# psweens/VAN-GAN

Measured on AMD Instinct MI355X. Metric: train Mvoxels/s (VanGan.train_step, 128^3 bf16), higher is better.
Workload: dtype bf16; 1 GPU; VanGan.train_step, 128x128x128 volumes, batch 1 per GPU (global 1), clDice on, disc noise+dropout on; parallelism=dp1

## Files before the change

van_gan_amd/csrc/vg_conv_common.h:

```cpp
#pragma once
#include "vg_gather.h"

struct ConvOut {
    int OD, OH, OW, ostr, ood, ooh, oow, BD, BH, BW, Cout;
    const void* wp; int Ktot, nchunks, kc_pad;
    const float* bias; const void* res; const float* rs; const float* rb; int tanh_out;
    int res1;
    int wdma;
    const void* wp_up; int nup;
    void* out; int out_f32, accumulate; float* sums;
    int w_lds;
    int dma;
    int xw;
    int dbg;
    int WRS;
    const void* bs_x0; const void* bs_x1; int bs_c0, bs_sh, bs_act, bs_pad, bs_D, bs_H, bs_W;
    const float* bs_sc; const float* bs_sf; const float* bs_mu; const float* bs_rs; const float* bs_ml;
    int ks; float* ks_part; unsigned* ks_cnt;
    char* scratch; long scratch_bytes;
    VgFin fin;
};
struct ConvCls {
    int ncls;
    int par;
// ... 97 lines not shown
            o1 = koff[min(s + 3, last) * 4 + kg];
            a0 = wfrag(min(s + 2, last));
#pragma unroll
            for (int i = 0; i < MW; ++i) b0[i] = *(const bf16x8*)(halo + rowbase[i] + o2);
            if (s + 1 >= ksteps) a1 = zero8;
            __builtin_amdgcn_sched_barrier(0);
#pragma unroll
            for (int i = 0; i < MW; ++i) acc[i] = VG_MFMA16(a1, b1[i], acc[i]);
            __builtin_amdgcn_sched_barrier(0);
        }
    }
}


bool vg_conv_thin_ok(const vg_conv_desc* d, const GatherIn& g, const ConvOut& k, const ConvCls& q, int np);
int vg_conv_thin_lds_bytes(const GatherIn& g, int np, int pl = 1, bool up = false, bool wdma = false);
int vg_launch_conv_thin(const GatherIn& g, const ConvOut& k, int np, hipStream_t s, float* red, bool& did_stats);
```

van_gan_amd/csrc/vg_conv_thin.hip:

```cpp
#include "vg_conv_common.h"
#include <stdio.h>

static int vg_ablate_knob(const char* key) {
    const int v = vg_tune(key, 0);
#ifdef VG_DEBUG_ABLATE
    return v;
#else
    if (v != 0) { fprintf(stderr, "libvangan_hip: VG_%s=%d is a timing-ablation knob of a -DVG_DEBUG_ABLATE build; this library refuses it\n", key, v); return -1; }
    return 0;
#endif
}
#include "vg_dma_common.h"
#include <type_traits>
#include <algorithm>
#include <cstdio>

#ifndef VG_THIN_WPE
#define VG_THIN_WPE 2
#endif
#ifndef VG_THIN_PF2
#define VG_THIN_PF2 0
#endif
#ifndef VG_THIN_PD
#define VG_THIN_PD 1
#endif
namespace {
constexpr int TW = 16, TH = 8, TD = 4;
constexpr int HW = 18, HH = 10, HD = 6;
constexpr int UNIT = 16;
constexpr int ROWB = HW * UNIT;
constexpr int DSB = HH * ROWB;
constexpr int PSB = ((HD * DSB + 255) / 256) * 256;
constexpr int HALO = 2 * PSB;
constexpr int KSTEPS = 14;
constexpr int KCPAD = 448;
}

__device__ __forceinline__ void lds_only_barrier() { asm volatile("s_waitcnt lgkmcnt(0)\n\ts_barrier" ::: "memory"); }

struct ThinItem { int hoff, cg; bool cv; const char* pc; const int* dt; };
struct ThinTab { const int* tab; int AL, NH, NW, od0, oh0, ow0; };
__device__ __forceinline__ void thin_axis_tables(const GatherIn& g, int* tab, int NH, int NW, int ND, int tid) {
    const int AL = NH + NW + ND, sh = g.shift0;
    for (int i = tid; i < 2 * AL; i += 256) {
        const int set = i >= AL ? 1 : 0, j = i - set * AL;
        if (set == 1 && g.c1 == 0) { tab[i] = -1; continue; }
        const int axis = j < NH ? 1 : (j < NH + NW ? 2 : 0);
        const int jj = axis == 1 ? j : (axis == 2 ? j - NH : j - NH - NW);
        const int n_ax = axis == 1 ? g.H : (axis == 2 ? g.W : g.D);
        int p = (axis == 1 ? g.tmin_h : (axis == 2 ? g.tmin_w : g.tmin_d)) + jj;
        const bool valid = resolve_pos(p, n_ax, g.pad_mode);
        long off;
        if (set == 0) {
            const int ps = p >> sh, Ws = g.W >> sh, Hs = g.H >> sh;
            off = axis == 1 ? (long)ps * Ws * g.c0 : (axis == 2 ? (long)ps * g.c0 : (long)ps * Hs * Ws * g.c0);
        } else off = axis == 1 ? (long)p * g.W * g.c1 : (axis == 2 ? (long)p * g.c1 : (long)p * g.H * g.W * g.c1);
        tab[i] = valid ? (int)(off * 2) : -1;
    }
}
template <bool PLAIN>
__device__ __forceinline__ ThinItem thin_item(const GatherIn& g, const int* ctab, const ThinTab& tt, const char* b0, const char* b1, int chunk, int item) {
    constexpr int NCOLS = HH * HW * 2, SEGL = HD / 2;
    ThinItem t;
    const int seg = item >= NCOLS ? 1 : 0, col = item - seg * NCOLS;
    const int e = ctab[2 * col];
    t.hoff = ctab[2 * col + 1] + seg * SEGL * DSB;
    const int hh = e & 1023, hw = (e >> 10) & 1023;
    t.cg = e >> 20;
    const int c = chunk * 16 + t.cg * 8;
    const bool from0 = c < g.c0;
    const int* rs = tt.tab + (from0 ? 0 : tt.AL);
    const int oh = rs[tt.oh0 + hh], ow = rs[tt.NH + tt.ow0 + hw];
    t.cv = !PLAIN || (c < g.Cin && (oh | ow) >= 0);
    t.pc = t.cv ? (from0 ? b0 + (size_t)c * 2 : b1 + (size_t)(c - g.c0) * 2) + (oh + ow) : b0;
    t.dt = rs + tt.NH + tt.NW + tt.od0 + seg * SEGL;
    return t;
}
template <int MODE>
__device__ __forceinline__ void thin_issue(const GatherIn& g, const int* ctab, const ThinTab& rt, int n, int chunk, int tid, Raw8<bf16_t> (&raw)[3][HD / 2]) {
    typedef bf16_t T;
    constexpr int NITEMS = 4 * HH * HW, SEGL = HD / 2;
    const int sh = g.shift0;
    const char* b0 = (const char*)g.src0 + (size_t)n * (g.D >> sh) * (g.H >> sh) * (g.W >> sh) * g.c0 * 2;
    const char* b1 = (const char*)g.src1 + (size_t)n * g.D * g.H * g.W * g.c1 * 2;
#pragma unroll
    for (int i = 0; i < 3; ++i) {
        const int item = tid + 256 * i;
        if (i < 2 || item < NITEMS) {
            const ThinItem t = thin_item<MODE == VG_STAGE_PLAIN>(g, ctab, rt, b0, b1, chunk, item);
#pragma unroll
            for (int k = 0; k < SEGL; ++k) raw_load(raw[i][k], (const T*)(t.pc + (unsigned)max(t.dt[k], 0)));
        }
    }
}
template <int MODE>
__device__ __forceinline__ void thin_commit(const GatherIn& g, char* halo, const float* scs, const int* ctab, const ThinTab& rt, int chunk, int tid,
                                            Raw8<bf16_t> (&raw)[3][HD / 2]) {
    typedef bf16_t T;
    constexpr bool plain = MODE == VG_STAGE_PLAIN;
    constexpr int NITEMS = 4 * HH * HW, SEGL = HD / 2;
#pragma unroll
    for (int i = 0; i < 3; ++i) {
        const int item = tid + 256 * i;
        if (i < 2 || item < NITEMS) {
            const ThinItem t = thin_item<plain>(g, ctab, rt, nullptr, nullptr, chunk, item);
            f32x2 sc[4], sf[4];
            if (!plain) {
#pragma unroll
                for (int j = 0; j < 4; ++j) {
                    sc[j] = (f32x2){scs[t.cg * 8 + 2 * j], scs[t.cg * 8 + 2 * j + 1]};
                    sf[j] = (f32x2){scs[16 + t.cg * 8 + 2 * j], scs[16 + t.cg * 8 + 2 * j + 1]};
                }
            }
#pragma unroll
            for (int k = 0; k < SEGL; ++k) {
                T* dst = (T*)(halo + t.hoff + k * DSB);
                if (plain) {
                    Raw8<T> r = raw[i][k];
                    raw_mask(r, t.cv && t.dt[k] >= 0);
                    *(Raw8<T>*)dst = r;
// ... 76 lines not shown
            for (int k = 0; k < 2; ++k) {
                float x[8];
                raw_unpack(raw[i][k], x);
#pragma unroll
                for (int j = 0; j < 4; ++j) {
                    f32x2 v = {x[2 * j], x[2 * j + 1]};
                    v = v * sc[j] + sf[j];
                    x[2 * j] = fmaxf(v[0], 0.f); x[2 * j + 1] = fmaxf(v[1], 0.f);
                }
                store8<bf16_t>((bf16_t*)(halo + hoff + k * DSB), x);
            }
        }
    }
}

template <int MODE, bool BIAS, bool RES, bool STATS, bool BSTAT = false, int NP = 1, int PL = 1, bool UP = false>
__global__ __launch_bounds__(256, VG_THIN_WPE) void conv_thin_kernel(const GatherIn g, const ConvOut p) {
    static_assert(PL == 1 || (NP == 1 && MODE == VG_STAGE_PLAIN && !BIAS && !RES && !STATS), "panel loop: plain data gradient only");
    static_assert(!UP || (MODE == VG_STAGE_RELU && !RES && !BSTAT && PL == 1 && NP == 1), "collapsed upsampled chunks: the decoder's first convolution, forward, one panel");
    typedef bf16_t T;
    extern __shared__ __attribute__((aligned(16))) char smem[];
    const int tid = threadIdx.x, lane = tid & 63, wave = __builtin_amdgcn_readfirstlane(tid >> 6);
    const int li = lane & 15, kg = lane >> 4;
    const int n = blockIdx.z, ntile = blockIdx.y;
    char* halo = smem;
    float* scs = (float*)(smem + HALO);
    float* stat = scs + 32;
    float* bsc = stat + 32 * NP * PL;
    float* ebs = bsc + 64 * NP * PL;
    int* tapb = (int*)(ebs + (NP > 1 ? 48 * NP : 0));
    int* utab = tapb + 32;
    constexpr int NCOLS = HH * HW * 2;
    int* xtab = utab + 2 * NCOLS;
    const int NHt = g.tiles_h * TH + 2, NWt = g.tiles_w * TW + 2, NDt = g.tiles_d * TD + 2;
    const int NHl = UP ? g.tiles_h * (TH / 2) + 2 : 0, NDl = UP ? g.tiles_d * (TD / 2) + 2 : 0;
    int* lowtab = xtab + 2 * (NHt + NWt + NDt);
    int* utu = lowtab + NHl + NDl;
    char* wlds = (char*)(utu + (UP ? 2 * UPCOLS + 16 : 0));
    const bool wdma = MODE == VG_STAGE_RELU && NP == 1 && PL == 1 && !UP && p.wdma;
    wlds = (char*)(((size_t)wlds + ((PL > 1 || wdma) ? 1023 : 15)) & ~(size_t)((PL > 1 || wdma) ? 1023 : 15));
    const int Ktot = p.Ktot, nchunks = p.nchunks;
    constexpr int WRS = KCPAD * 2 + 16;
    const int cop = ntile * 16 * NP * PL;

    build_column_table(g, utab, tid);
    if (tid < 32 * NP * PL) stat[tid] = 0.f;
    if constexpr (NP > 1 && (BIAS || RES)) {
        if (tid < 16 * NP) {
            const int c = cop + tid;
            ebs[tid] = BIAS ? p.bias[c] : 0.f;
            if (RES) { ebs[16 * NP + tid] = p.rs[n * p.Cout + c]; ebs[32 * NP + tid] = p.rb[n * p.Cout + c]; }
        }
    }
    if constexpr (BSTAT) {
        constexpr int CW = 16 * NP * PL;
        if (tid < CW) {
            const int nc = n * p.Cout + cop + tid;
            const float rs = p.bs_rs[nc];
            bsc[tid] = p.bs_sc[nc]; bsc[CW + tid] = p.bs_sf[nc]; bsc[2 * CW + tid] = rs; bsc[3 * CW + tid] = -p.bs_mu[nc] * rs;
        }
    }
    if (tid < 27) tapb[tid] = (g.td[tid] - g.tmin_d) * DSB + (g.th[tid] - g.tmin_h) * ROWB + (g.tw[tid] - g.tmin_w) * UNIT;
    auto load_weights = [&](int chunk) {
        const char* src = (const char*)p.wp + ((size_t)cop * Ktot + (size_t)chunk * KCPAD) * 2;
        constexpr int NU = 16 * NP * 56, NK = (NU + 255) / 256;
        f32x4 v[NK];
        int tid = threadIdx.x;
        if constexpr (UP) asm volatile("" : "+v"(tid));
#pragma unroll
        for (int k = 0; k < NK; ++k) {
            const int u = min(tid + k * 256, NU - 1);
            const int r = u / 56, c = u - r * 56;
            v[k] = *(const __attribute__((address_space(1))) f32x4*)(uintptr_t)(src + (size_t)r * Ktot * 2 + c * 16);
        }
#pragma unroll
        for (int k = 0; k < NK; ++k) {
            const int u = tid + k * 256;
// ... 15 lines not shown
    };
    if constexpr (PL > 1) dma_weights(0, 0); else if constexpr (!UP) { if (wdma) dma_weights(0, 0, 0); else load_weights(0); }
    const int wbase = li * WRS + kg * 16;
    const int wbase_up = li * WRSU + kg * 16;
    const int co0 = cop + 4 * kg;
    float s1[NP * PL][4], s2[NP * PL][4];
    f32x2 e_b[NP][2], e_rs[NP][2], e_rb[NP][2];
#pragma unroll
    for (int q = 0; q < NP * PL; ++q)
#pragma unroll
        for (int r = 0; r < 4; ++r) { s1[q][r] = 0.f; s2[q][r] = 0.f; }
#pragma unroll
    for (int q = 0; q < NP; ++q) {
        const int c = co0 + 16 * q;
        e_b[q][0] = (f32x2){0.f, 0.f}; e_b[q][1] = e_b[q][0];
        if (BIAS && NP == 1) { e_b[q][0] = (f32x2){p.bias[c], p.bias[c + 1]}; e_b[q][1] = (f32x2){p.bias[c + 2], p.bias[c + 3]}; }
        if (RES && NP == 1) {
            e_rs[q][0] = (f32x2){p.rs[n * p.Cout + c], p.rs[n * p.Cout + c + 1]}; e_rs[q][1] = (f32x2){p.rs[n * p.Cout + c + 2], p.rs[n * p.Cout + c + 3]};
            e_rb[q][0] = (f32x2){p.rb[n * p.Cout + c], p.rb[n * p.Cout + c + 1]}; e_rb[q][1] = (f32x2){p.rb[n * p.Cout + c + 2], p.rb[n * p.Cout + c + 3]};
        }
    }
    const T* b_x[NP]; int b_cs[NP], b_sh[NP]; float b_slope = 1.f;
#pragma unroll
    for (int q = 0; q < NP; ++q) { b_x[q] = nullptr; b_cs[q] = 0; b_sh[q] = 0; }
    auto bstat_panel = [&](const int pn16) {
#pragma unroll
        for (int q = 0; q < NP; ++q) {
            const int c = co0 + 16 * q + pn16;
            const bool lo = c < p.bs_c0;
            b_sh[q] = lo ? p.bs_sh : 0; b_cs[q] = lo ? p.bs_c0 : p.Cout - p.bs_c0;
            b_x[q] = (lo ? (const T*)p.bs_x0 + c : (const T*)p.bs_x1 + (c - p.bs_c0))
                     + (size_t)n * (p.bs_D >> b_sh[q]) * (p.bs_H >> b_sh[q]) * (p.bs_W >> b_sh[q]) * b_cs[q];
// ... 5 lines not shown
    }
    const int cst = cop + 8 * (kg >> 1);
    const int jodd = kg & 1;

    const int tiles_per_n = g.tiles_d * g.tiles_h * g.tiles_w;
    int t0 = blockIdx.x, tstep = gridDim.x, tend = tiles_per_n;
    if (p.xw) {
        const int slab = (tiles_per_n + 7) >> 3, xcd = blockIdx.x & 7;
        t0 = xcd * slab + ((int)blockIdx.x >> 3); tstep = gridDim.x >> 3; tend = min(tiles_per_n, (xcd + 1) * slab);
    }
    int gs_w, gs_h, gs_d;
    { int t = tstep; gs_w = t % g.tiles_w; t /= g.tiles_w; gs_h = t % g.tiles_h; gs_d = t / g.tiles_h; }
    int ti_w, ti_h, ti_d;
    { int t = t0; ti_w = t % g.tiles_w; t /= g.tiles_w; ti_h = t % g.tiles_h; ti_d = t / g.tiles_h; }
    if (nchunks == 1) stage_scale_shift(g, scs, n, 0, tid);
    thin_axis_tables(g, xtab, NHt, NWt, NDt, tid);
    if constexpr (UP) { build_up_table(utu, tid); thin_up_axis_tables(g, lowtab, NHl, NDl, tid); }
    lds_only_barrier();
    auto tabat = [&](int od0_, int oh0_, int ow0_) { return ThinTab{xtab, NHt + NWt + NDt, NHt, NWt, od0_, oh0_, ow0_}; };
    int boff[KSTEPS];
    {
        const int rowbase = wave * DSB + li * UNIT;
#pragma unroll
        for (int s = 0; s < KSTEPS; ++s) {
            int G = 4 * s + kg; if (G > 53) G = 53;
            boff[s] = rowbase + tapb[G >> 1] + (G & 1) * PSB;
        }
    }

    int* tapu = utu + 2 * UPCOLS;
    if constexpr (UP) { if (tid < 12) { const int cdh = tid / 3, cw = tid - cdh * 3; tapu[tid] = (cdh >> 1) * DSB + (cdh & 1) * ROWB + cw * UNIT; } }
    const int pd_cls = UP ? (wave & 1) * 2 : 0;
    constexpr int CLSB = 16 * NP * WRSU;
    auto load_weights_up = [&](int chunk) {
        const char* src = (const char*)p.wp_up + ((size_t)chunk * 4 * p.Cout + cop) * KUP * 2;
        constexpr int NU = 4 * 16 * NP * 24, NK = (NU + 255) / 256;
        f32x4 v[NK];
// ... 6 lines not shown
            v[k] = *(const __attribute__((address_space(1))) f32x4*)(uintptr_t)(src + ((size_t)cls * p.Cout + rr) * KUP * 2 + c * 16);
        }
#pragma unroll
        for (int k = 0; k < NK; ++k) {
            const int u = tl + k * 256;
            if (u < NU) { const int r = u / 24, c = u - r * 24; *(f32x4*)(wlds + r * WRSU + c * 16) = v[k]; }
        }
    };
    auto uptab = [&](int od0_, int oh0_, int ow0_) { return ThinUpTab{xtab + NHt + ow0_, lowtab + (oh0_ >> 1), lowtab + NHl + (od0_ >> 1)}; };
    typedef const __attribute__((address_space(3))) bf16x8 lds_frag;
    int it = 0;
    constexpr bool PF = MODE == VG_STAGE_RELU && (NP == 1 || VG_THIN_PF2);
    Raw8<T> raw[3][HD / 2];
    if (PF && t0 < tend) {
        if constexpr (UP) thin_issue_up<MODE>(g, utu, uptab(ti_d * TD, ti_h * TH, ti_w * TW), n, 0, tid, raw);
        else thin_issue<MODE>(g, utab, tabat(ti_d * TD, ti_h * TH, ti_w * TW), n, 0, tid, raw);
    }
    bf16x4 bxp[(BSTAT && NP == 1) ? 8 : 1];
    bf16x4 bxn[(BSTAT && PL > 1) ? 8 : 1];
    for (int tile = t0; tile < tend; tile += tstep, ++it) {
        const int od0 = ti_d * TD, oh0 = ti_h * TH, ow0 = ti_w * TW;
        ti_w += gs_w; if (ti_w >= g.tiles_w) { ti_w -= g.tiles_w; ++ti_h; }
        ti_h += gs_h; if (ti_h >= g.tiles_h) { ti_h -= g.tiles_h; ++ti_d; }
        ti_d += gs_d;
        const bool more = tile + tstep < tend;
        f32x4 acc[NP][8];
#pragma unroll
        for (int q = 0; q < NP; ++q)
#pragma unroll
            for (int j = 0; j < 8; ++j) acc[q][j] = (f32x4){0.f, 0.f, 0.f, 0.f};
        auto issue_bxp = [&]() {
// ... 45 lines not shown
                __builtin_amdgcn_sched_barrier(0);
            }
        };
        if constexpr (PL == 1)
        for (int chunk = 0; chunk < nchunks; ++chunk) {
            const bool upc = UP && chunk < p.nup;
            if (it | chunk) lds_only_barrier();
            if (nchunks > 1) {
                stage_scale_shift(g, scs, n, chunk, tid);
                if constexpr (UP) { if (upc) load_weights_up(chunk); else load_weights(chunk); }
                else if ((it | chunk) && !wdma) load_weights(chunk);
                lds_only_barrier();
            }
            if constexpr (UP) {
                if (upc) { if (!PF) thin_issue_up<MODE>(g, utu, uptab(od0, oh0, ow0), n, chunk, tid, raw); thin_commit_up(halo, scs, utu, tid, raw); }
                else { if (!PF) thin_issue<MODE>(g, utab, tabat(od0, oh0, ow0), n, chunk, tid, raw); thin_commit<MODE>(g, halo, scs, utab, tabat(od0, oh0, ow0), chunk, tid, raw); }
            } else {
            if (!PF) thin_issue<MODE>(g, utab, tabat(od0, oh0, ow0), n, chunk, tid, raw);
            thin_commit<MODE>(g, halo, scs, utab, tabat(od0, oh0, ow0), chunk, tid, raw);
            }
            if (wdma) __builtin_amdgcn_s_waitcnt(0x0F70);
            lds_only_barrier();
            if (PF) {
                if constexpr (UP) {
                    if (chunk + 1 < nchunks) {
                        if (chunk + 1 < p.nup) thin_issue_up<MODE>(g, utu, uptab(od0, oh0, ow0), n, chunk + 1, tid, raw);
                        else thin_issue<MODE>(g, utab, tabat(od0, oh0, ow0), n, chunk + 1, tid, raw);
                    } else if (more) thin_issue_up<MODE>(g, utu, uptab(ti_d * TD, ti_h * TH, ti_w * TW), n, 0, tid, raw);
                } else {
                if (chunk + 1 < nchunks) thin_issue<MODE>(g, utab, tabat(od0, oh0, ow0), n, chunk + 1, tid, raw);
                else if (more) thin_issue<MODE>(g, utab, tabat(ti_d * TD, ti_h * TH, ti_w * TW), n, 0, tid, raw);
                }
            }
            const int wuse = it * nchunks + chunk;
            if (wdma && (chunk + 1 < nchunks || more)) dma_weights(0, (wuse + 1) & 1, chunk + 1 < nchunks ? chunk + 1 : 0);
            if constexpr (UP) {
                if (upc) {
                    const char* wbu = wlds + pd_cls * CLSB + wbase_up;
                    int boff_up[KSUP];
                    {
                        const int upbase = ((wave + 1) >> 1) * DSB + li * UNIT;
#pragma unroll
                        for (int s_ = 0; s_ < KSUP; ++s_) { const int G = 4 * s_ + kg; boff_up[s_] = upbase + tapu[G >> 1] + (G & 1) * PSB; }
                    }
                    bf16x8 ae[2][NP], ao[2][NP], bu[2][5];
#pragma unroll
// ... 11 lines not shown
#pragma unroll
                            for (int r = 0; r < 5; ++r) bu[(s_ + 1) & 1][r] = *(lds_frag*)(halo + boff_up[s_ + 1] + r * ROWB);
                        }
                        __builtin_amdgcn_sched_barrier(0);
#pragma unroll
                        for (int q = 0; q < NP; ++q)
#pragma unroll
                            for (int j = 0; j < 8; ++j) acc[q][j] = VG_MFMA16((j & 1) ? ao[s_ & 1][q] : ae[s_ & 1][q], bu[s_ & 1][(j + 1) >> 1], acc[q][j]);
                        __builtin_amdgcn_sched_barrier(0);
                    }
                    continue;
                }
            }
            const char* wb = wlds + wbase + (wdma ? (wuse & 1) * WBUF : 0);
            constexpr int PD = VG_THIN_PD, NB = PD + 1;
            if constexpr (NP == 1) {
                bf16x8 a[NB][NP], b[NB][8];
#pragma unroll
                for (int u = 0; u < PD; ++u) {
#pragma unroll
                    for (int q = 0; q < NP; ++q) a[u][q] = *(lds_frag*)(wb + q * 16 * WRS + u * 64);
#pragma unroll
                    for (int j = 0; j < 8; ++j) b[u][j] = *(lds_frag*)(halo + boff[u] + j * ROWB);
                }
#pragma unroll
                for (int s = 0; s < KSTEPS; ++s) {
                    if (s + PD < KSTEPS) {
#pragma unroll
                        for (int q = 0; q < NP; ++q) a[(s + PD) % NB][q] = *(lds_frag*)(wb + q * 16 * WRS + (s + PD) * 64);
#pragma unroll
                        for (int j = 0; j < 8; ++j) b[(s + PD) % NB][j] = *(lds_frag*)(halo + boff[s + PD] + j * ROWB);
// ... 32 lines not shown
                }
            }
        }
        const int od = od0 + wave, ow = ow0 + li;
        const size_t rowpitch = (size_t)p.BW * p.Cout;
        const size_t obase = (((size_t)(n * p.BD + od + p.ood) * p.BH + oh0 + p.ooh) * p.BW + ow + p.oow) * p.Cout;
        const bool full = od0 + TD <= p.OD && oh0 + TH <= p.OH && ow0 + TW <= p.OW;
        auto epilogue = [&](auto masked_tag, const int pn16) {
            constexpr bool MASKED = decltype(masked_tag)::value;
            const bool dw_ok = !MASKED || (od < p.OD && ow < p.OW);
            const int nrow = MASKED ? p.OH - oh0 : TH;
            typedef __attribute__((ext_vector_type(2))) unsigned u32x2;
            typedef __attribute__((ext_vector_type(4))) unsigned u32x4;
#pragma unroll
            for (int q = 0; q < NP; ++q) {
            T* const optr = (T*)p.out + obase + cst + 16 * q + pn16;
            const T* const rptr = RES ? (const T*)p.res + obase + co0 + 16 * q : nullptr;
            const float* const r1ptr = RES ? (const float*)p.res + (((size_t)(n * p.BD + od + p.ood) * p.BH + oh0 + p.ooh) * p.BW + ow + p.oow) : nullptr;
            f32x2 eb[2], ers[2], erb[2];
            if constexpr (NP == 1) { eb[0] = e_b[0][0]; eb[1] = e_b[0][1]; if (RES) { ers[0] = e_rs[0][0]; ers[1] = e_rs[0][1]; erb[0] = e_rb[0][0]; erb[1] = e_rb[0][1]; } }
            else {
                const float* eq = ebs + 4 * kg + 16 * q;
                if (BIAS) { const f32x4 t = *(const f32x4*)eq; eb[0] = (f32x2){t[0], t[1]}; eb[1] = (f32x2){t[2], t[3]}; }
                if (RES) {
                    const f32x4 t = *(const f32x4*)(eq + 16 * NP), u = *(const f32x4*)(eq + 32 * NP);
                    ers[0] = (f32x2){t[0], t[1]}; ers[1] = (f32x2){t[2], t[3]}; erb[0] = (f32x2){u[0], u[1]}; erb[1] = (f32x2){u[2], u[3]};
                }
            }
            bf16x4 bx[BSTAT ? 8 : 1];
            f32x2 b_sc[2], b_sf[2], b_rs[2], b_nm[2];
            if (BSTAT) {
                constexpr int CW = 16 * NP * PL;
                const float* bq = bsc + 4 * kg + 16 * q + pn16;
                const f32x4 c_sc = *(const f32x4*)bq, c_sf = *(const f32x4*)(bq + CW), c_rs = *(const f32x4*)(bq + 2 * CW), c_nm = *(const f32x4*)(bq + 3 * CW);
                b_sc[0] = (f32x2){c_sc[0], c_sc[1]}; b_sc[1] = (f32x2){c_sc[2], c_sc[3]}; b_sf[0] = (f32x2){c_sf[0], c_sf[1]}; b_sf[1] = (f32x2){c_sf[2], c_sf[3]};
                b_rs[0] = (f32x2){c_rs[0], c_rs[1]}; b_rs[1] = (f32x2){c_rs[2], c_rs[3]};
                b_nm[0] = (f32x2){c_nm[0], c_nm[1]}; b_nm[1] = (f32x2){c_nm[2], c_nm[3]};
                auto fold = [&](int qq, int nn) { int i = qq - p.bs_pad; i = i < 0 ? -i : i; i = i >= nn ? 2 * nn - 2 - i : i; return min(max(i, 0), nn - 1); };
                const int XH = p.bs_H >> b_sh[q], XW = p.bs_W >> b_sh[q];
                const int id = fold(od + p.ood, p.bs_D) >> b_sh[q], iw = fold(ow + p.oow, p.bs_W) >> b_sh[q];
                const T* xcol = b_x[q] + ((size_t)id * XH * XW + iw) * b_cs[q];
#pragma unroll
                for (int j = 0; j < 8; ++j) {
                    if constexpr (NP == 1) bx[j] = bxp[j];
                    else {
                        const int ih = fold(oh0 + j + p.ooh, p.bs_H) >> b_sh[q];
                        bx[j] = *(const __attribute__((address_space(1))) bf16x4*)(uintptr_t)(xcol + (size_t)ih * XW * b_cs[q]);
                    }
                }
            }
            constexpr int RRN = NP == 1 ? 8 : 4;
            bf16x4 rr[RES ? 8 : 1];
#pragma unroll
            for (int jp = 0; jp < 8; jp += 2) {
                if constexpr (RES) {
                    if (jp % RRN == 0) {
#pragma unroll
                        for (int j = jp; j < jp + RRN; ++j) {
                            const bool ok = !MASKED || (dw_ok && j < nrow);
                            if (NP == 1 && p.res1) {
                                const float xv = ld_global(ok ? r1ptr + (size_t)j * p.BW : r1ptr);
                                rr[j] = __builtin_bit_cast(bf16x4, (u32x2){__float_as_uint(xv), 0u});
                            } else
                            rr[j] = *(const __attribute__((address_space(1))) bf16x4*)(uintptr_t)(ok ? rptr + j * rowpitch : rptr);
                        }
                    }
// ... 27 lines not shown
                        const f32x2 pre0 = x0 * b_sc[0] + b_sf[0], pre1 = x1 * b_sc[1] + b_sf[1];
                        const f32x2 d0 = {pre0[0] > 0.f ? 1.f : b_slope, pre0[1] > 0.f ? 1.f : b_slope};
                        const f32x2 d1 = {pre1[0] > 0.f ? 1.f : b_slope, pre1[1] > 0.f ? 1.f : b_slope};
                        const f32x2 dn0 = q0 * d0, dn1 = q1 * d1;
                        const f32x2 xh0 = x0 * b_rs[0] + b_nm[0], xh1 = x1 * b_rs[1] + b_nm[1];
                        f32x2 a0 = {s1[q][0], s1[q][1]}, a1 = {s1[q][2], s1[q][3]}, c0 = {s2[q][0], s2[q][1]}, c1 = {s2[q][2], s2[q][3]};
                        a0 += dn0; a1 += dn1; c0 += dn0 * xh0; c1 += dn1 * xh1;
                        s1[q][0] = a0[0]; s1[q][1] = a0[1]; s1[q][2] = a1[0]; s1[q][3] = a1[1]; s2[q][0] = c0[0]; s2[q][1] = c0[1]; s2[q][2] = c1[0]; s2[q][3] = c1[1];
                    }
                }
                const u32x2 wa = __builtin_bit_cast(u32x2, pk[0]), wb2 = __builtin_bit_cast(u32x2, pk[1]);
                const u32x2 x0 = __builtin_amdgcn_permlane16_swap(wa[0], wb2[0], false, false);
                const u32x2 x1 = __builtin_amdgcn_permlane16_swap(wa[1], wb2[1], false, false);
                const u32x4 outv = {x0[0], x1[0], x0[1], x1[1]};
                const int j = jp + jodd;
                if (!MASKED || (dw_ok && j < nrow)) *(u32x4*)(optr + j * rowpitch) = outv;
                if constexpr (BSTAT && PL > 1) { __builtin_amdgcn_sched_barrier(0); bxn[jp] = bx_row(jp); bxn[jp + 1] = bx_row(jp + 1); __builtin_amdgcn_sched_barrier(0); }
            }
            }
        };
        if constexpr (PL == 1) { if (full) epilogue(std::false_type{}, 0); else epilogue(std::true_type{}, 0); }
        else {
            if (it) lds_only_barrier();
            if constexpr (BSTAT) {
                if (it == 0) {
                    bx_prepare(0, od0, oh0, ow0);
#pragma unroll
                    for (int j = 0; j < 8; ++j) bxn[j] = bx_row(j);
                }
            }
            if (!(p.dbg & 16) || it == 0) {
            thin_issue<MODE>(g, utab, tabat(od0, oh0, ow0), n, 0, tid, raw);
            thin_commit<MODE>(g, halo, scs, utab, tabat(od0, oh0, ow0), 0, tid, raw);
            }
#pragma unroll 1
            for (int pn = 0; pn < PL; ++pn) {
                const int use = it * PL + pn;
                if (use == 0) asm volatile("s_waitcnt vmcnt(0)" ::: "memory");
                lds_only_barrier();
                if (pn + 1 < PL || more) dma_weights(pn + 1 < PL ? pn + 1 : 0, (use + 1) & 1);
#pragma unroll
                for (int j = 0; j < 8; ++j) acc[0][j] = (f32x4){0.f, 0.f, 0.f, 0.f};
                if (!(p.dbg & 4)) mfma_panel(wlds + (use & 1) * WBUF + wbase);
                __builtin_amdgcn_s_waitcnt(0x0F70);
                asm volatile("" ::: "memory");
                if constexpr (BSTAT) {
#pragma unroll
                    for (int j = 0; j < 8; ++j) asm volatile("v_mov_b64 %0, %1" : "=&v"(bxp[j]) : "v"(bxn[j]));
// ... 21 lines not shown
                float a = s1[q][r], b = s2[q][r];
#pragma unroll
                for (int o = 1; o < 16; o <<= 1) { a += __shfl_xor(a, o); b += __shfl_xor(b, o); }
                if (li == 0) { atomicAdd(&stat[(16 * q + 4 * kg + r) * 2], a); atomicAdd(&stat[(16 * q + 4 * kg + r) * 2 + 1], b); }
            }
        __syncthreads();
        if (tid < 32 * NP * PL) {
            const int co = cop + (tid >> 1);
            const int stripe = blockIdx.x & (VG_STRIPES - 1);
            if (co < p.Cout) atomicAdd(&p.sums[(((size_t)stripe * gridDim.z + n) * p.Cout + co) * 2 + (tid & 1)], stat[tid]);
        }
        if constexpr (STATS && (NP == 2 || !RES)) { if (p.fin.ticket) vg_fin_tail(p.fin, p.sums, gridDim.z, p.Cout, gridDim.x * gridDim.y * gridDim.z, (int*)stat); }
    }
}

int vg_conv_thin_lds_bytes(const GatherIn& g, int np, int pl, bool up, bool wdma) {
    const int AL = (g.tiles_h * TH + 2) + (g.tiles_w * TW + 2) + (g.tiles_d * TD + 2);
    int head = HALO + (32 + 32 * np * pl + 64 * np * pl + (np > 1 ? 48 * np : 0) + 32) * 4 + (2 * HH * HW * 2 + 2 * AL) * 4;
    if (pl > 1 || wdma) return head + 1024 + 2 * 15 * 1024;
    if (up) {
        head += (g.tiles_h * (TH / 2) + 2 + g.tiles_d * (TD / 2) + 2 + 2 * UPCOLS + 16) * 4;
        return head + 16 + std::max(16 * np * (KCPAD * 2 + 16), 4 * 16 * np * WRSU);
    }
    return head + 16 + 16 * np * (KCPAD * 2 + 16);
}

bool vg_conv_thin_ok(const vg_conv_desc* d, const GatherIn& g, const ConvOut& k, const ConvCls& q, int np) {
    if (!vg_tune("CONV_THIN", 1)) return false;
    if (d->f32 || d->noise || q.ncls != 1 || d->istr != 1 || d->ostr != 1 || d->CK != 16 || d->ntaps != 27 || d->wpack) return false;
    if ((d->c_src0 + d->c_src1) % 16 || (d->Cout % (16 * np)) || d->tanh_out || d->accumulate || d->out_f32) return false;
    if (g.lean != VG_STAGE_PLAIN && g.lean != VG_STAGE_RELU) return false;
    if (!g.planar || g.HW != HW || g.HH != HH || g.HD != HD || g.HWp != HW || g.HHp != HH || g.DS != DSB || g.PSB != PSB) return false;
    if ((1 << g.twl) != TW || (1 << g.thl) != TH || (1 << g.tdl) != TD) return false;
    if (d->res && (d->bias == nullptr)) return false;
    if (d->res_c1 && np != 1) return false;
    if (k.Ktot != k.nchunks * KCPAD) return false;
    for (int i = 0; i < 27; ++i)
        if (d->tap_d[i] - g.tmin_d > 2 || d->tap_h[i] - g.tmin_h > 2 || d->tap_w[i] - g.tmin_w > 2) return false;
    if (np > 1) {
        const long wgs = (long)g.tiles_d * g.tiles_h * g.tiles_w * (d->Cout / (16 * np)) * d->N;
        if (!vg_tune("CONV_THIN2", 1) || wgs < vg_tune("CONV_THIN2_MINWG", 96)) return false;
    }
    return true;
}

template <int MODE, bool BIAS, bool RES, bool STATS, bool BSTAT, int NP, int PL = 1, bool UP = false>
static int launch_thin_np(const GatherIn& g, const ConvOut& k, int lds, hipStream_t s) {
    static bool attr_set = false;
    if (!attr_set) {
        (void)hipFuncSetAttribute((const void*)conv_thin_kernel<MODE, BIAS, RES, STATS, BSTAT, NP, PL, UP>, hipFuncAttributeMaxDynamicSharedMemorySize, VG_LDS_LIMIT);
        attr_set = true;
    }
    int per_cu = 2;
    if (lds > 0 && VG_LDS_LIMIT / lds < per_cu) per_cu = VG_LDS_LIMIT / lds;
    if (per_cu < 1) per_cu = 1;
    const int tiles = g.tiles_d * g.tiles_h * g.tiles_w;
    const int ny = k.Cout / (16 * NP * PL);
    const int wg = vg_tune("CONV_THIN_WGS", 0) > 0 ? vg_tune("CONV_THIN_WGS", 0) : 256 * per_cu;
    int bx = wg / (ny * g.N); if (bx < 1) bx = 1; if (bx > tiles) bx = tiles;
    ConvOut k2 = k; k2.xw = 0; k2.dbg = PL > 1 ? vg_ablate_knob("THIN_DBG") : 0;
    if (k2.dbg < 0) return VG_EINVAL;
    if (vg_tune("CONV_THIN_XCD", 1) && bx >= 16 && tiles >= 4 * bx) { bx &= ~7; k2.xw = 1; }
    char name[96];
    snprintf(name, sizeof name, "%s<m%%d,b%%d,r%%d,s%%d%s%s%s>|walk%%d|ch%%d", NP == 2 ? "conv_thin2" : "conv_thin", BSTAT ? (k.bs_x1 ? ",bs2" : ",bs1") : "", PL > 1 ? ",pl" : "", UP ? ",up" : "");
    if (vg_dry(name, MODE, (int)BIAS, (int)RES, (int)STATS, tiles > bx ? 1 : 0, k.nchunks > 1 ? (k.wdma ? 2 : 1) : 0)) return VG_OK;
    const bool fin_here = STATS && k2.fin.ticket && k2.sums && ((NP == 2 && vg_tune("CONV_THIN2_FIN", 1)) || (NP == 1 && !RES && vg_tune("CONV_THIN1_FIN", 1)));
    if (!fin_here) k2.fin.ticket = nullptr;
    if constexpr (!UP) k2.nup = 0;
    hipLaunchKernelGGL((conv_thin_kernel<MODE, BIAS, RES, STATS, BSTAT, NP, PL, UP>), dim3(bx, ny, g.N), dim3(256), lds, s, g, k2);
    if (fin_here) vg_fin_done = true;
    return vg_check_launch();
}
template <int MODE, bool BIAS, bool RES, bool STATS, bool BSTAT = false>
static int launch_thin(const GatherIn& g, const ConvOut& k, int np, hipStream_t s) {
    if constexpr (BSTAT && MODE == VG_STAGE_PLAIN) {
        const int lds3 = vg_conv_thin_lds_bytes(g, 1, 3);
        if (np == 1 && k.Cout == 48 && k.nchunks == 1 && 2 * lds3 <= VG_LDS_LIMIT && vg_tune("CONV_THIN_PL", 1))
            return launch_thin_np<MODE, BIAS, RES, STATS, BSTAT, 1, 3>(g, k, lds3, s);
    }
    if constexpr (MODE == VG_STAGE_RELU && BIAS && !RES && !BSTAT) {
        if (k.nup > 0 && k.nup < k.nchunks && vg_tune("CONV_THIN_UP", 0)) {
            const int ldsu = vg_conv_thin_lds_bytes(g, np, 1, true);
            if (2 * ldsu <= VG_LDS_LIMIT) {
                if (np == 1) return launch_thin_np<MODE, BIAS, RES, STATS, BSTAT, 1, 1, true>(g, k, ldsu, s);
            }
        }
    }
    if constexpr (MODE == VG_STAGE_RELU && !BSTAT) {
        const int ldsw = vg_conv_thin_lds_bytes(g, 1, 1, false, true);
        if (np == 1 && k.nchunks > 1 && 2 * ldsw <= VG_LDS_LIMIT && vg_tune("CONV_THIN_WDMA", 1)) {
            ConvOut kw = k; kw.wdma = 1;
            return launch_thin_np<MODE, BIAS, RES, STATS, BSTAT, 1>(g, kw, ldsw, s);
        }
    }
    const int lds = vg_conv_thin_lds_bytes(g, np);
    if (lds > VG_LDS_LIMIT) return VG_ELDS;
    if constexpr (!BSTAT) { if (np == 2) return launch_thin_np<MODE, BIAS, RES, STATS, BSTAT, 2>(g, k, lds, s); }
    return np == 1 ? launch_thin_np<MODE, BIAS, RES, STATS, BSTAT, 1>(g, k, lds, s) : VG_EINVAL;
}

int vg_launch_conv_thin(const GatherIn& g, const ConvOut& k, int np, hipStream_t s, float* red, bool& did_stats) {
    const bool st = k.sums != nullptr;
    if (g.lean == VG_STAGE_PLAIN) {
        if (np == 1 && red && k.bs_x0 && !k.bs_ml && k.bs_sc && k.bias == nullptr && k.res == nullptr && !st && (k.bs_c0 % 16) == 0 && (k.bs_c0 == k.Cout || k.bs_x1)
            && k.OD == k.BD && k.OH == k.BH && k.OW == k.BW && !k.ood && !k.ooh && !k.oow && vg_tune("CONV_BSTAT", 1)) {
            ConvOut k2 = k; k2.sums = red;
            const int rc = launch_thin<VG_STAGE_PLAIN, false, false, false, true>(g, k2, np, s);
            did_stats = rc == VG_OK && !vg_dry_on();
            return rc;
        }
        if (k.bias == nullptr && k.res == nullptr && !st) return launch_thin<VG_STAGE_PLAIN, false, false, false>(g, k, np, s);
// ... 273 lines not shown
```

Measured before the change: 123.8 Mvoxels/s.

## Add three-workgroups-per-CU thin conv variant with packed tables and slimmer MFMA loop

Adds a WPE=3 instantiation of the thin convolution kernel that targets three 256-thread workgroups per CU. To fit the LDS budget it packs the column table into one int per column, builds one axis-table set when there is no second input, and reuses the bias staging area. It also replaces the register-heavy precomputed per-step offsets with a lean two-half-step MFMA loop that reads tap offsets from LDS. The goal is more latency hiding for one-panel convolutions. The cost is fewer registers per wave, a different output row mapping and a weight-DMA path that is turned off for this variant.

Result: no change. 124.9 Mvoxels/s (median of 6 runs) (+0.9%).

```diff
diff --git a/van_gan_amd/csrc/vg_conv_common.h b/van_gan_amd/csrc/vg_conv_common.h
--- a/van_gan_amd/csrc/vg_conv_common.h
+++ b/van_gan_amd/csrc/vg_conv_common.h
@@ -135,5 +135,5 @@
 
 
 bool vg_conv_thin_ok(const vg_conv_desc* d, const GatherIn& g, const ConvOut& k, const ConvCls& q, int np);
-int vg_conv_thin_lds_bytes(const GatherIn& g, int np, int pl = 1, bool up = false, bool wdma = false);
+int vg_conv_thin_lds_bytes(const GatherIn& g, int np, int pl = 1, bool up = false, bool wdma = false, int wpe = 2);
 int vg_launch_conv_thin(const GatherIn& g, const ConvOut& k, int np, hipStream_t s, float* red, bool& did_stats);
diff --git a/van_gan_amd/csrc/vg_conv_thin.hip b/van_gan_amd/csrc/vg_conv_thin.hip
--- a/van_gan_amd/csrc/vg_conv_thin.hip
+++ b/van_gan_amd/csrc/vg_conv_thin.hip
@@ -15,9 +15,6 @@
 #include <algorithm>
 #include <cstdio>
 
-#ifndef VG_THIN_WPE
-#define VG_THIN_WPE 2
-#endif
 #ifndef VG_THIN_PF2
 #define VG_THIN_PF2 0
 #endif
@@ -40,9 +37,9 @@
 
 struct ThinItem { int hoff, cg; bool cv; const char* pc; const int* dt; };
 struct ThinTab { const int* tab; int AL, NH, NW, od0, oh0, ow0; };
-__device__ __forceinline__ void thin_axis_tables(const GatherIn& g, int* tab, int NH, int NW, int ND, int tid) {
+__device__ __forceinline__ void thin_axis_tables(const GatherIn& g, int* tab, int NH, int NW, int ND, int tid, int nsets = 2) {
     const int AL = NH + NW + ND, sh = g.shift0;
-    for (int i = tid; i < 2 * AL; i += 256) {
+    for (int i = tid; i < nsets * AL; i += 256) {
         const int set = i >= AL ? 1 : 0, j = i - set * AL;
         if (set == 1 && g.c1 == 0) { tab[i] = -1; continue; }
         const int axis = j < NH ? 1 : (j < NH + NW ? 2 : 0);
@@ -58,15 +55,23 @@
         tab[i] = valid ? (int)(off * 2) : -1;
     }
 }
-template <bool PLAIN>
+__device__ __forceinline__ void build_column_table_packed(const GatherIn& g, int* ctab, int tid) {
+    constexpr int NV = HH * HW;
+    for (int col = tid; col < 2 * NV; col += 256) {
+        const int cg = col / NV, v = col - cg * NV;
+        const int hh = v / HW, hw = v - hh * HW;
+        ctab[col] = (cg * g.CS + (hh * g.HWp + halo_pos_w(g, hw)) * g.VS) | (hh << 16) | (hw << 20) | (cg << 25);
+    }
+}
+template <bool PLAIN, bool PK = false>
 __device__ __forceinline__ ThinItem thin_item(const GatherIn& g, const int* ctab, const ThinTab& tt, const char* b0, const char* b1, int chunk, int item) {
     constexpr int NCOLS = HH * HW * 2, SEGL = HD / 2;
     ThinItem t;
     const int seg = item >= NCOLS ? 1 : 0, col = item - seg * NCOLS;
-    const int e = ctab[2 * col];
-    t.hoff = ctab[2 * col + 1] + seg * SEGL * DSB;
-    const int hh = e & 1023, hw = (e >> 10) & 1023;
-    t.cg = e >> 20;
+    const int e = PK ? ctab[col] : ctab[2 * col];
+    t.hoff = (PK ? (e & 0xffff) : ctab[2 * col + 1]) + seg * SEGL * DSB;
+    const int hh = PK ? (e >> 16) & 15 : e & 1023, hw = PK ? (e >> 20) & 31 : (e >> 10) & 1023;
+    t.cg = PK ? e >> 25 : e >> 20;
     const int c = chunk * 16 + t.cg * 8;
     const bool from0 = c < g.c0;
     const int* rs = tt.tab + (from0 ? 0 : tt.AL);
@@ -76,7 +81,7 @@
     t.dt = rs + tt.NH + tt.NW + tt.od0 + seg * SEGL;
     return t;
 }
-template <int MODE>
+template <int MODE, bool PK = false>
 __device__ __forceinline__ void thin_issue(const GatherIn& g, const int* ctab, const ThinTab& rt, int n, int chunk, int tid, Raw8<bf16_t> (&raw)[3][HD / 2]) {
     typedef bf16_t T;
     constexpr int NITEMS = 4 * HH * HW, SEGL = HD / 2;
@@ -87,13 +92,13 @@
     for (int i = 0; i < 3; ++i) {
         const int item = tid + 256 * i;
         if (i < 2 || item < NITEMS) {
-            const ThinItem t = thin_item<MODE == VG_STAGE_PLAIN>(g, ctab, rt, b0, b1, chunk, item);
+            const ThinItem t = thin_item<MODE == VG_STAGE_PLAIN, PK>(g, ctab, rt, b0, b1, chunk, item);
 #pragma unroll
             for (int k = 0; k < SEGL; ++k) raw_load(raw[i][k], (const T*)(t.pc + (unsigned)max(t.dt[k], 0)));
         }
     }
 }
-template <int MODE>
+template <int MODE, bool PK = false>
 __device__ __forceinline__ void thin_commit(const GatherIn& g, char* halo, const float* scs, const int* ctab, const ThinTab& rt, int chunk, int tid,
                                             Raw8<bf16_t> (&raw)[3][HD / 2]) {
     typedef bf16_t T;
@@ -103,7 +108,7 @@
     for (int i = 0; i < 3; ++i) {
         const int item = tid + 256 * i;
         if (i < 2 || item < NITEMS) {
-            const ThinItem t = thin_item<plain>(g, ctab, rt, nullptr, nullptr, chunk, item);
+            const ThinItem t = thin_item<plain, PK>(g, ctab, rt, nullptr, nullptr, chunk, item);
             f32x2 sc[4], sf[4];
             if (!plain) {
 #pragma unroll
@@ -210,8 +215,9 @@
     }
 }
 
-template <int MODE, bool BIAS, bool RES, bool STATS, bool BSTAT = false, int NP = 1, int PL = 1, bool UP = false>
-__global__ __launch_bounds__(256, VG_THIN_WPE) void conv_thin_kernel(const GatherIn g, const ConvOut p) {
+template <int MODE, bool BIAS, bool RES, bool STATS, bool BSTAT = false, int NP = 1, int PL = 1, bool UP = false, int WPE = 2>
+__global__ __launch_bounds__(256, WPE) void conv_thin_kernel(const GatherIn g, const ConvOut p) {
+    static_assert(WPE == 2 || (WPE == 3 && NP == 1 && PL == 1 && !UP), "three workgroups per CU: one-panel instances without panel loop or upsampled chunks");
     static_assert(PL == 1 || (NP == 1 && MODE == VG_STAGE_PLAIN && !BIAS && !RES && !STATS), "panel loop: plain data gradient only");
     static_assert(!UP || (MODE == VG_STAGE_RELU && !RES && !BSTAT && PL == 1 && NP == 1), "collapsed upsampled chunks: the decoder's first convolution, forward, one panel");
     typedef bf16_t T;
@@ -223,25 +229,28 @@
     float* scs = (float*)(smem + HALO);
     float* stat = scs + 32;
     float* bsc = stat + 32 * NP * PL;
-    float* ebs = bsc + 64 * NP * PL;
-    int* tapb = (int*)(ebs + (NP > 1 ? 48 * NP : 0));
+    constexpr bool EBL = NP > 1 || (WPE == 3 && !BSTAT);
+    float* ebs = (WPE == 3 && !BSTAT) ? bsc : bsc + 64 * NP * PL;
+    int* tapb = (int*)(bsc + 64 * NP * PL + (NP > 1 ? 48 * NP : 0));
     int* utab = tapb + 32;
     constexpr int NCOLS = HH * HW * 2;
-    int* xtab = utab + 2 * NCOLS;
+    constexpr bool PK = WPE == 3;
+    int* xtab = utab + (PK ? 1 : 2) * NCOLS;
     const int NHt = g.tiles_h * TH + 2, NWt = g.tiles_w * TW + 2, NDt = g.tiles_d * TD + 2;
     const int NHl = UP ? g.tiles_h * (TH / 2) + 2 : 0, NDl = UP ? g.tiles_d * (TD / 2) + 2 : 0;
-    int* lowtab = xtab + 2 * (NHt + NWt + NDt);
+    const int nsets = (UP || g.c1) ? 2 : 1;
+    int* lowtab = xtab + nsets * (NHt + NWt + NDt);
     int* utu = lowtab + NHl + NDl;
     char* wlds = (char*)(utu + (UP ? 2 * UPCOLS + 16 : 0));
-    const bool wdma = MODE == VG_STAGE_RELU && NP == 1 && PL == 1 && !UP && p.wdma;
+    const bool wdma = MODE == VG_STAGE_RELU && NP == 1 && PL == 1 && !UP && WPE == 2 && p.wdma;
     wlds = (char*)(((size_t)wlds + ((PL > 1 || wdma) ? 1023 : 15)) & ~(size_t)((PL > 1 || wdma) ? 1023 : 15));
-    const int Ktot = p.Ktot, nchunks = p.nchunks;
+    const int Ktot = p.Ktot, nchunks = (WPE == 3 && BSTAT) ? 1 : p.nchunks;
     constexpr int WRS = KCPAD * 2 + 16;
     const int cop = ntile * 16 * NP * PL;
 
-    build_column_table(g, utab, tid);
+    if constexpr (PK) build_column_table_packed(g, utab, tid); else build_column_table(g, utab, tid);
     if (tid < 32 * NP * PL) stat[tid] = 0.f;
-    if constexpr (NP > 1 && (BIAS || RES)) {
+    if constexpr (EBL && (BIAS || RES)) {
         if (tid < 16 * NP) {
             const int c = cop + tid;
             ebs[tid] = BIAS ? p.bias[c] : 0.f;
@@ -256,7 +265,7 @@
             bsc[tid] = p.bs_sc[nc]; bsc[CW + tid] = p.bs_sf[nc]; bsc[2 * CW + tid] = rs; bsc[3 * CW + tid] = -p.bs_mu[nc] * rs;
         }
     }
-    if (tid < 27) tapb[tid] = (g.td[tid] - g.tmin_d) * DSB + (g.th[tid] - g.tmin_h) * ROWB + (g.tw[tid] - g.tmin_w) * UNIT;
+    if (tid < 28) { const int t = min(tid, 26); tapb[tid] = (g.td[t] - g.tmin_d) * DSB + (g.th[t] - g.tmin_h) * ROWB + (g.tw[t] - g.tmin_w) * UNIT; }
     auto load_weights = [&](int chunk) {
         const char* src = (const char*)p.wp + ((size_t)cop * Ktot + (size_t)chunk * KCPAD) * 2;
         constexpr int NU = 16 * NP * 56, NK = (NU + 255) / 256;
@@ -302,8 +311,8 @@
     for (int q = 0; q < NP; ++q) {
         const int c = co0 + 16 * q;
         e_b[q][0] = (f32x2){0.f, 0.f}; e_b[q][1] = e_b[q][0];
-        if (BIAS && NP == 1) { e_b[q][0] = (f32x2){p.bias[c], p.bias[c + 1]}; e_b[q][1] = (f32x2){p.bias[c + 2], p.bias[c + 3]}; }
-        if (RES && NP == 1) {
+        if (BIAS && !EBL) { e_b[q][0] = (f32x2){p.bias[c], p.bias[c + 1]}; e_b[q][1] = (f32x2){p.bias[c + 2], p.bias[c + 3]}; }
+        if (RES && !EBL) {
             e_rs[q][0] = (f32x2){p.rs[n * p.Cout + c], p.rs[n * p.Cout + c + 1]}; e_rs[q][1] = (f32x2){p.rs[n * p.Cout + c + 2], p.rs[n * p.Cout + c + 3]};
             e_rb[q][0] = (f32x2){p.rb[n * p.Cout + c], p.rb[n * p.Cout + c + 1]}; e_rb[q][1] = (f32x2){p.rb[n * p.Cout + c + 2], p.rb[n * p.Cout + c + 3]};
         }
@@ -339,13 +348,15 @@
     int ti_w, ti_h, ti_d;
     { int t = t0; ti_w = t % g.tiles_w; t /= g.tiles_w; ti_h = t % g.tiles_h; ti_d = t / g.tiles_h; }
     if (nchunks == 1) stage_scale_shift(g, scs, n, 0, tid);
-    thin_axis_tables(g, xtab, NHt, NWt, NDt, tid);
+    thin_axis_tables(g, xtab, NHt, NWt, NDt, tid, nsets);
     if constexpr (UP) { build_up_table(utu, tid); thin_up_axis_tables(g, lowtab, NHl, NDl, tid); }
     lds_only_barrier();
-    auto tabat = [&](int od0_, int oh0_, int ow0_) { return ThinTab{xtab, NHt + NWt + NDt, NHt, NWt, od0_, oh0_, ow0_}; };
-    int boff[KSTEPS];
-    {
-        const int rowbase = wave * DSB + li * UNIT;
+    auto tabat = [&](int od0_, int oh0_, int ow0_) { return ThinTab{xtab, (nsets - 1) * (NHt + NWt + NDt), NHt, NWt, od0_, oh0_, ow0_}; };
+    const int rowbase = wave * DSB + li * UNIT;
+    const int* tapl = tapb + (kg >> 1);
+    int boff[WPE == 3 ? 1 : KSTEPS];
+    if constexpr (WPE == 3) boff[0] = 0;
+    else {
 #pragma unroll
         for (int s = 0; s < KSTEPS; ++s) {
             int G = 4 * s + kg; if (G > 53) G = 53;
@@ -382,7 +393,7 @@
     Raw8<T> raw[3][HD / 2];
     if (PF && t0 < tend) {
         if constexpr (UP) thin_issue_up<MODE>(g, utu, uptab(ti_d * TD, ti_h * TH, ti_w * TW), n, 0, tid, raw);
-        else thin_issue<MODE>(g, utab, tabat(ti_d * TD, ti_h * TH, ti_w * TW), n, 0, tid, raw);
+        else thin_issue<MODE, PK>(g, utab, tabat(ti_d * TD, ti_h * TH, ti_w * TW), n, 0, tid, raw);
     }
     bf16x4 bxp[(BSTAT && NP == 1) ? 8 : 1];
     bf16x4 bxn[(BSTAT && PL > 1) ? 8 : 1];
@@ -458,10 +469,10 @@
             }
             if constexpr (UP) {
                 if (upc) { if (!PF) thin_issue_up<MODE>(g, utu, uptab(od0, oh0, ow0), n, chunk, tid, raw); thin_commit_up(halo, scs, utu, tid, raw); }
-                else { if (!PF) thin_issue<MODE>(g, utab, tabat(od0, oh0, ow0), n, chunk, tid, raw); thin_commit<MODE>(g, halo, scs, utab, tabat(od0, oh0, ow0), chunk, tid, raw); }
+                else { if (!PF) thin_issue<MODE, PK>(g, utab, tabat(od0, oh0, ow0), n, chunk, tid, raw); thin_commit<MODE, PK>(g, halo, scs, utab, tabat(od0, oh0, ow0), chunk, tid, raw); }
             } else {
-            if (!PF) thin_issue<MODE>(g, utab, tabat(od0, oh0, ow0), n, chunk, tid, raw);
-            thin_commit<MODE>(g, halo, scs, utab, tabat(od0, oh0, ow0), chunk, tid, raw);
+            if (!PF) thin_issue<MODE, PK>(g, utab, tabat(od0, oh0, ow0), n, chunk, tid, raw);
+            thin_commit<MODE, PK>(g, halo, scs, utab, tabat(od0, oh0, ow0), chunk, tid, raw);
             }
             if (wdma) __builtin_amdgcn_s_waitcnt(0x0F70);
             lds_only_barrier();
@@ -469,11 +480,11 @@
                 if constexpr (UP) {
                     if (chunk + 1 < nchunks) {
                         if (chunk + 1 < p.nup) thin_issue_up<MODE>(g, utu, uptab(od0, oh0, ow0), n, chunk + 1, tid, raw);
-                        else thin_issue<MODE>(g, utab, tabat(od0, oh0, ow0), n, chunk + 1, tid, raw);
+                        else thin_issue<MODE, PK>(g, utab, tabat(od0, oh0, ow0), n, chunk + 1, tid, raw);
                     } else if (more) thin_issue_up<MODE>(g, utu, uptab(ti_d * TD, ti_h * TH, ti_w * TW), n, 0, tid, raw);
                 } else {
-                if (chunk + 1 < nchunks) thin_issue<MODE>(g, utab, tabat(od0, oh0, ow0), n, chunk + 1, tid, raw);
-                else if (more) thin_issue<MODE>(g, utab, tabat(ti_d * TD, ti_h * TH, ti_w * TW), n, 0, tid, raw);
+                if (chunk + 1 < nchunks) thin_issue<MODE, PK>(g, utab, tabat(od0, oh0, ow0), n, chunk + 1, tid, raw);
+                else if (more) thin_issue<MODE, PK>(g, utab, tabat(ti_d * TD, ti_h * TH, ti_w * TW), n, 0, tid, raw);
                 }
             }
             const int wuse = it * nchunks + chunk;
@@ -515,7 +526,37 @@
             }
             const char* wb = wlds + wbase + (wdma ? (wuse & 1) * WBUF : 0);
             constexpr int PD = VG_THIN_PD, NB = PD + 1;
-            if constexpr (NP == 1) {
+            if constexpr (NP == 1 && WPE == 3) {
+                bf16x8 a[2], b[2][4];
+                int tv[2], bo;
+                const int lanep = rowbase + (kg & 1) * PSB;
+                typedef const __attribute__((address_space(3))) char lds_char;
+                lds_char* const wl = (lds_char*)wb;
+                lds_char* const hl = (lds_char*)halo;
+                tv[0] = tapl[0]; tv[1] = tapl[2];
+                a[0] = *(lds_frag*)wl;
+                bo = lanep + tv[0];
+#pragma unroll
+                for (int j = 0; j < 4; ++j) b[0][j] = *(lds_frag*)(hl + bo + j * ROWB);
+#pragma unroll
+                for (int hs = 0; hs < 2 * KSTEPS; ++hs) {
+                    const int s = hs >> 1, h = hs & 1;
+                    if (hs + 1 < 2 * KSTEPS) {
+                        const int s2 = (hs + 1) >> 1, h2 = (hs + 1) & 1;
+                        if (h2 == 0) {
+                            a[s2 & 1] = *(lds_frag*)(wl + s2 * 64);
+                            bo = (s2 == KSTEPS - 1 ? rowbase + (kg ? PSB : 0) : lanep) + tv[s2 & 1];
+                            if (s2 + 1 < KSTEPS) tv[(s2 + 1) & 1] = tapl[2 * (s2 + 1)];
+                        }
+#pragma unroll
+                        for (int j = 0; j < 4; ++j) b[(hs + 1) & 1][j] = *(lds_frag*)(hl + bo + (4 * h2 + j) * ROWB);
+                    }
+                    __builtin_amdgcn_sched_barrier(0);
+#pragma unroll
+                    for (int j = 0; j < 4; ++j) acc[0][4 * h + j] = VG_MFMA16(a[s & 1], b[hs & 1][j], acc[0][4 * h + j]);
+                    __builtin_amdgcn_sched_barrier(0);
+                }
+            } else if constexpr (NP == 1) {
                 bf16x8 a[NB][NP], b[NB][8];
 #pragma unroll
                 for (int u = 0; u < PD; ++u) {
@@ -578,11 +619,11 @@
             typedef __attribute__((ext_vector_type(4))) unsigned u32x4;
 #pragma unroll
             for (int q = 0; q < NP; ++q) {
-            T* const optr = (T*)p.out + obase + cst + 16 * q + pn16;
+            T* const optr = (T*)p.out + obase + cst + 16 * q + pn16 + (WPE == 3 ? jodd * rowpitch : (size_t)0);
             const T* const rptr = RES ? (const T*)p.res + obase + co0 + 16 * q : nullptr;
             const float* const r1ptr = RES ? (const float*)p.res + (((size_t)(n * p.BD + od + p.ood) * p.BH + oh0 + p.ooh) * p.BW + ow + p.oow) : nullptr;
             f32x2 eb[2], ers[2], erb[2];
-            if constexpr (NP == 1) { eb[0] = e_b[0][0]; eb[1] = e_b[0][1]; if (RES) { ers[0] = e_rs[0][0]; ers[1] = e_rs[0][1]; erb[0] = e_rb[0][0]; erb[1] = e_rb[0][1]; } }
+            if constexpr (!EBL) { eb[0] = e_b[0][0]; eb[1] = e_b[0][1]; if (RES) { ers[0] = e_rs[0][0]; ers[1] = e_rs[0][1]; erb[0] = e_rb[0][0]; erb[1] = e_rb[0][1]; } }
             else {
                 const float* eq = ebs + 4 * kg + 16 * q;
                 if (BIAS) { const f32x4 t = *(const f32x4*)eq; eb[0] = (f32x2){t[0], t[1]}; eb[1] = (f32x2){t[2], t[3]}; }
@@ -613,7 +654,7 @@
                     }
                 }
             }
-            constexpr int RRN = NP == 1 ? 8 : 4;
+            constexpr int RRN = (NP == 1 && WPE == 2) ? 8 : 4;
             bf16x4 rr[RES ? 8 : 1];
 #pragma unroll
             for (int jp = 0; jp < 8; jp += 2) {
@@ -671,7 +712,7 @@
                 const u32x2 x1 = __builtin_amdgcn_permlane16_swap(wa[1], wb2[1], false, false);
                 const u32x4 outv = {x0[0], x1[0], x0[1], x1[1]};
                 const int j = jp + jodd;
-                if (!MASKED || (dw_ok && j < nrow)) *(u32x4*)(optr + j * rowpitch) = outv;
+                if (!MASKED || (dw_ok && j < nrow)) *(u32x4*)(optr + (WPE == 3 ? jp : j) * rowpitch) = outv;
                 if constexpr (BSTAT && PL > 1) { __builtin_amdgcn_sched_barrier(0); bxn[jp] = bx_row(jp); bxn[jp + 1] = bx_row(jp + 1); __builtin_amdgcn_sched_barrier(0); }
             }
             }
@@ -687,8 +728,8 @@
                 }
             }
             if (!(p.dbg & 16) || it == 0) {
-            thin_issue<MODE>(g, utab, tabat(od0, oh0, ow0), n, 0, tid, raw);
-            thin_commit<MODE>(g, halo, scs, utab, tabat(od0, oh0, ow0), 0, tid, raw);
+            thin_issue<MODE, PK>(g, utab, tabat(od0, oh0, ow0), n, 0, tid, raw);
+            thin_commit<MODE, PK>(g, halo, scs, utab, tabat(od0, oh0, ow0), 0, tid, raw);
             }
 #pragma unroll 1
             for (int pn = 0; pn < PL; ++pn) {
@@ -740,9 +781,9 @@
     }
 }
 
-int vg_conv_thin_lds_bytes(const GatherIn& g, int np, int pl, bool up, bool wdma) {
+int vg_conv_thin_lds_bytes(const GatherIn& g, int np, int pl, bool up, bool wdma, int wpe) {
     const int AL = (g.tiles_h * TH + 2) + (g.tiles_w * TW + 2) + (g.tiles_d * TD + 2);
-    int head = HALO + (32 + 32 * np * pl + 64 * np * pl + (np > 1 ? 48 * np : 0) + 32) * 4 + (2 * HH * HW * 2 + 2 * AL) * 4;
+    int head = HALO + (32 + 32 * np * pl + 64 * np * pl + (np > 1 ? 48 * np : 0) + 32) * 4 + ((wpe == 3 ? 1 : 2) * HH * HW * 2 + (g.c1 ? 2 : 1) * AL) * 4;
     if (pl > 1 || wdma) return head + 1024 + 2 * 15 * 1024;
     if (up) {
         head += (g.tiles_h * (TH / 2) + 2 + g.tiles_d * (TD / 2) + 2 + 2 * UPCOLS + 16) * 4;
@@ -770,14 +811,14 @@
     return true;
 }
 
-template <int MODE, bool BIAS, bool RES, bool STATS, bool BSTAT, int NP, int PL = 1, bool UP = false>
+template <int MODE, bool BIAS, bool RES, bool STATS, bool BSTAT, int NP, int PL = 1, bool UP = false, int WPE = 2>
 static int launch_thin_np(const GatherIn& g, const ConvOut& k, int lds, hipStream_t s) {
     static bool attr_set = false;
     if (!attr_set) {
-        (void)hipFuncSetAttribute((const void*)conv_thin_kernel<MODE, BIAS, RES, STATS, BSTAT, NP, PL, UP>, hipFuncAttributeMaxDynamicSharedMemorySize, VG_LDS_LIMIT);
+        (void)hipFuncSetAttribute((const void*)conv_thin_kernel<MODE, BIAS, RES, STATS, BSTAT, NP, PL, UP, WPE>, hipFuncAttributeMaxDynamicSharedMemorySize, VG_LDS_LIMIT);
         attr_set = true;
     }
-    int per_cu = 2;
+    int per_cu = WPE;
     if (lds > 0 && VG_LDS_LIMIT / lds < per_cu) per_cu = VG_LDS_LIMIT / lds;
     if (per_cu < 1) per_cu = 1;
     const int tiles = g.tiles_d * g.tiles_h * g.tiles_w;
@@ -793,10 +834,12 @@
     const bool fin_here = STATS && k2.fin.ticket && k2.sums && ((NP == 2 && vg_tune("CONV_THIN2_FIN", 1)) || (NP == 1 && !RES && vg_tune("CONV_THIN1_FIN", 1)));
     if (!fin_here) k2.fin.ticket = nullptr;
     if constexpr (!UP) k2.nup = 0;
-    hipLaunchKernelGGL((conv_thin_kernel<MODE, BIAS, RES, STATS, BSTAT, NP, PL, UP>), dim3(bx, ny, g.N), dim3(256), lds, s, g, k2);
+    hipLaunchKernelGGL((conv_thin_kernel<MODE, BIAS, RES, STATS, BSTAT, NP, PL, UP, WPE>), dim3(bx, ny, g.N), dim3(256), lds, s, g, k2);
     if (fin_here) vg_fin_done = true;
     return vg_check_launch();
 }
+template <int MODE, bool BIAS, bool RES, bool STATS, bool BSTAT>
+static constexpr bool thin_wpe3() { return MODE == VG_STAGE_RELU || !BIAS; }
 template <int MODE, bool BIAS, bool RES, bool STATS, bool BSTAT = false>
 static int launch_thin(const GatherIn& g, const ConvOut& k, int np, hipStream_t s) {
     if constexpr (BSTAT && MODE == VG_STAGE_PLAIN) {
@@ -821,6 +864,10 @@
     }
     const int lds = vg_conv_thin_lds_bytes(g, np);
     if (lds > VG_LDS_LIMIT) return VG_ELDS;
+    if constexpr (thin_wpe3<MODE, BIAS, RES, STATS, BSTAT>()) {
+        const int lds3 = vg_conv_thin_lds_bytes(g, 1, 1, false, false, 3);
+        if (np == 1 && 3 * ((lds3 + 1279) / 1280) * 1280 <= VG_LDS_LIMIT && (!BSTAT || k.nchunks == 1) && vg_tune("CONV_THIN_WPC", 3) >= 3) return launch_thin_np<MODE, BIAS, RES, STATS, BSTAT, 1, 1, false, 3>(g, k, lds3, s);
+    }
     if constexpr (!BSTAT) { if (np == 2) return launch_thin_np<MODE, BIAS, RES, STATS, BSTAT, 2>(g, k, lds, s); }
     return np == 1 ? launch_thin_np<MODE, BIAS, RES, STATS, BSTAT, 1>(g, k, lds, s) : VG_EINVAL;
 }
```
